# pvangoor/eqf_vio

Measured on AMD Instinct MI355X. Metric: EqF propagate+update steps/sec at N=200 landmarks (fp32); 1-GPU + 8-GPU batch, higher is better.
Workload: dtype f64

## Files before the change

### eqf_vio_amd/csrc/eqf_capi.hip

```cpp
#include <hip/hip_runtime.h>

#include <algorithm>
#include <cmath>
#include <cstdio>
#include <cstdlib>
#include <cstring>
#include <type_traits>
#include <vector>

#include "../../include/eqf_vio_amd_debug.h"
#include "eqf_churn.hpp"
#include "eqf_dense.hpp"
#include "eqf_device.hpp"
#include "eqf_propagate.hpp"
#include "eqf_burst.hpp"
#include "eqf_chol64.hpp"
#include "eqf_resident.hpp"
#include "eqf_update.hpp"
#include "eqf_i8.hpp"
#include "eqf_local.hpp"
#include "eqf_innov.hpp"
#include "eqf_factor.hpp"
#include "eqf_nees.hpp"
#include "eqf_clone.hpp"
#include "eqf_frame.hpp"
#include "eqf_sample.hpp"
#include "eqf_sample_host.hpp"
#include "eqf_blocks.hpp"
#include "eqf_blocks_host.hpp"
#include "eqf_linear.hpp"
#include "eqf_linear_host.hpp"
#include "eqf_mixture.hpp"
#include "eqf_mixture_host.hpp"
#include "eqf_mergecost.hpp"
#include "eqf_mergecost_host.hpp"
#include "eqf_forecast.hpp"
#include "eqf_forecast_host.hpp"
#include "eqf_score.hpp"
#include "eqf_score_host.hpp"
#include "eqf_lift.hpp"
#include "eqf_lift_host.hpp"
#include "eqf_mapedit.hpp"
#include "eqf_mapedit_host.hpp"
#include "eqf_schmidt.hpp"
#include "eqf_schmidt_host.hpp"

using namespace eqf;

#define HIPC(expr)                                                                              \
    do {                                                                                        \
        hipError_t e_ = (expr);                                                                 \
        if (e_ != hipSuccess) {                                                                 \
            std::fprintf(stderr, "eqf_vio_amd: %s failed: %s (%s:%d)\n", #expr, hipGetErrorString(e_), __FILE__, __LINE__); \
            return EQF_ERR_HIP;                                                                 \
        }                                                                                       \
    } while (0)

namespace {
constexpr int kRing = 64;

struct ProfPair {
    int cls, key;
    hipEvent_t a, b;
};
struct ProfSample {
    int key;
    float ms;
};

void launchI8Dd(int slices, const I8DdArgs& a, const UpdArgs* u, int nCt, hipStream_t st) {
    UpdArgs uu{};
    if (u) uu = *u;
    i8WithSlices(slices, [&](auto s) {
        hipLaunchKernelGGL((k_i8dd_split<s>), dim3(nCt + (u ? 1 : 0), a.B), dim3(256), 0, st, a, uu, u ? 1 : 0);
// ... 134 lines not shown
    bool neesLdsSet = false;
    double *dSampZ = nullptr, *dSampE = nullptr;
    int sampRows = 0;
    char *hSampSmall = nullptr, *dSampSmall = nullptr;
    hipEvent_t evSamp = nullptr;
    char *hLinSmall = nullptr, *dLinSmall = nullptr;
    double *dLinWs = nullptr, *dLinOut = nullptr;
    hipEvent_t evLin = nullptr;
    char *hBlkSmall = nullptr, *dBlkSmall = nullptr;
    size_t blkSmallBytes = 0, blkWsDoubles = 0, blkWiInts = 0;
    double *dBlkWs = nullptr, *dBlkOut = nullptr;
    int* dBlkWi = nullptr;
    hipEvent_t evBlk = nullptr;
    bool blkLdsSet = false;
    int liftOpt = 0;
    bool liftCalled = false, liftLdsSet = false;
    double *dLiftRec = nullptr, *dLiftE = nullptr, *dLiftD = nullptr;
    int* dLiftBad = nullptr;
    ClonePair *hClonePairs = nullptr, *dClonePairs = nullptr;
    int clonePairsCap = 0;
    char* dCloneSmall = nullptr;
    hipEvent_t evCloneSrc = nullptr, evCloneDone = nullptr;
    double* dMixWs = nullptr;
    char *hMixTab = nullptr, *dMixTab = nullptr;
    size_t mixTabBytes = 0;
    int mixLaunches = 0;
    hipEvent_t evMix = nullptr;
    int innovStats = 0;
    double* dInnov = nullptr;
    int resTickets = 0;
    double *dGammaPart = nullptr, *dG11Part = nullptr;
    ResRole* dRoles = nullptr;
    int rolesN = -1, rolesCount = 0;
    int rolesFront = 0;
    int dropRole[4] = {-1, 0, 0, 0};
    bool prof = false;
    std::vector<ProfPair> profPairs;
    std::vector<hipEvent_t> evPool;
    long long profCount[EQF_PROF_CLASSES] = {};
    double profMs[EQF_PROF_CLASSES] = {};
    std::vector<ProfSample> profSamples[EQF_PROF_CLASSES];
    double profOverheadMs = 0.0;
    ImuRec *hFcImu = nullptr, *dFcImu = nullptr;
    double *dFcRec = nullptr, *dFcOut = nullptr, *hFcOut = nullptr;
    char* dMcWs = nullptr;
    int mcChunkCap = 0, mcChunkOpt = 0;
    char* dMcItems = nullptr;
    size_t mcItemCap = 0;
    char* dScWs = nullptr;
    int scChunkCap = 0, scChunkOpt = 0;
    char* dScTab = nullptr;
    size_t scTabBytes = 0;
    bool scoreLdsSet = false;
    char *hMapEdit = nullptr, *dMapEdit = nullptr;
    hipEvent_t evMapEdit = nullptr;
    char *hSch = nullptr, *dSch = nullptr;
    char* hSchDev = nullptr;
    hipEvent_t evSch = nullptr;
    bool schLdsSet = false;
};

namespace {

template <typename F>
int profiled(eqf_filter* f, int cls, F&& launch, int key = 0) {
    if (!f->prof) {
// ... 374 lines not shown
        if (status) status[b] = st;
    }
}

UpdArgs makeUpdArgs(eqf_filter* f, const double* bearings, long long bearStride, const int* perm) {
    UpdArgs a{};
    a.g = f->g[f->pG];
    a.p0 = f->p0;
    a.lmc = f->lmc;
    a.Q = f->Q[f->pG];
    a.Sin = f->Sigma[f->pS];
    a.Sout = f->Sigma[f->pS ^ 1];
    a.sigmaStride = f->sigmaStride;
    a.cap = f->cap;
    a.ld = f->ld;
    a.bearings = bearings;
    a.bearStride = bearStride;
    a.perm = perm;
    a.SA = f->SA; a.SL = f->SL; a.YW = f->YW; a.YO = f->YO;
    a.ldS = f->ldS; a.ldY = f->ldY; a.strideS = f->strideS; a.strideY = f->strideY;
    a.EA = f->EA; a.EL = f->EL; a.ZW = f->ZW; a.ZO = f->ZO;
    a.ldE = f->ldE; a.ldZ = f->ldZ; a.strideE = f->strideE; a.strideZ = f->strideZ;
    a.dbgDelta = f->dbgDelta;
    a.dbgGamma = f->dbgGamma;
    a.dbgGammaTot = f->dbgGammaTot;
    a.red = f->red;
    a.errflag = f->errflag;
    a.resCounters = f->dResCounters;
    a.prm = f->prm;
    a.csInBurst = f->csValid ? 1 : 0;
    return a;
}

int buildRoles(eqf_filter* f, int Nmax, bool fold, int front = 0) {
    const int nbS = roundUp(sDim(Nmax), kSB) / kSB, nbE = roundUp(eDim(Nmax), kSB) / kSB, wtS = roundUp(yCols(Nmax), kSB) / kSB;
    const int key = (fold ? 1 << 30 : 0) | (front << 27) | (nbS << 18) | (nbE << 9) | wtS;
    if (f->rolesN == key) return EQF_OK;
    std::vector<ResRole> r;
    if (fold) {
        r.push_back({1, 6, 0, 0});
        r.push_back({0, 6, 0, 0});
        for (int s = 0; s < std::min(front, nbE - 1); ++s) {
            r.push_back({1, 0, s + 1, 0});
            for (int R = s + 2; R < nbE; ++R) r.push_back({1, 1, R, s});
        }
    }
    f->rolesFront = fold ? int(r.size()) : 0;
    if (!(fold && front > 0)) f->rolesFront = 0;
    for (int s = 0; s < std::max(nbS, nbE); ++s)
        for (int kind = 1; kind >= 0; --kind) {
            const int nb = kind ? nbE : nbS, wt = kind ? 1 : wtS;
            if (s >= nb) continue;
            const bool moved = fold && kind == 1 && s < front;
            if (s + 1 < nb && !moved) r.push_back({kind, 0, s + 1, 0});
            for (int R = s + 2; R < nb && !moved; ++R) r.push_back({kind, 1, R, s});
            for (int t = 0; t < wt; ++t) r.push_back({kind, 2, t, s});
        }
    if (f->dropRole[0] >= 0)
        for (auto& q : r)
            if (q.kind == f->dropRole[0] && q.role == f->dropRole[1] && q.R == f->dropRole[2] && q.C == f->dropRole[3]) q.R = 1 << 20;
    HIPC(hipStreamSynchronize(f->stream));
    hipFree(f->dRoles);
    f->dRoles = nullptr;
    int rc = dmalloc(&f->dRoles, r.size());
    if (rc) return rc;
    HIPC(hipMemcpy(f->dRoles, r.data(), sizeof(ResRole) * r.size(), hipMemcpyHostToDevice));
    f->rolesN = key;
    f->rolesCount = int(r.size());
    return EQF_OK;
}

struct UpdateShape {
    int nbS, nbE, wtS, nv;
    int wpb, nvPad, lmBlocks, eBlocks;
    size_t prepLds;
    bool occ2Prep;
    bool embed;
    bool splitChain;
    bool resident;
    bool residentFits;
    bool fold;
    int front;
    bool pipeHeads, occ2;
    int eFromSigma;
    bool small;
    int ddNt, ddTiles;
    int i8Slices;
    bool tailLaunch, tailLift;
};

int updateShape(eqf_filter* f, int Nmax, UpdateShape& s) {
    const int B = f->B;
    const bool f64 = f->precision != EQF_PRECISION_F32;
    s.nbS = roundUp(sDim(Nmax), kSB) / kSB, s.nbE = roundUp(eDim(Nmax), kSB) / kSB, s.wtS = roundUp(yCols(Nmax), kSB) / kSB;
    s.nv = kLm0 + 3 * Nmax;
    const int mp = roundUp(sDim(Nmax), kSB), nep = roundUp(eDim(Nmax), kSB);
    s.nvPad = roundUp(std::min(s.nv, kLm0 + 3 * kPrepLmChunk), 16);
    const size_t perWave = size_t(2) * s.nvPad * sizeof(double);
    s.wpb = int(std::min<size_t>(4, (150 * 1024) / perWave));
    if (s.wpb < 1) return EQF_ERR_CAPACITY;
// ... 47 lines not shown
#endif
    const int fullLds = int(sizeof(Step64Lds));
    auto fn = [](auto* kernel) { return reinterpret_cast<const void*>(kernel); };
    const struct { const void* fn; int bytes; } table[] = {
        {fn(&k_update_prep64<float, false>), prepLds},
        {fn(&k_update_prep64<double, false>), prepLds},
        {fn(&k_update_prep64<float, true>), prepLds},
        {fn(&k_update_prep64<double, true>), prepLds},
        {fn(&k_chol_resident<float, false>), fullLds},
        {fn(&k_chol_resident<double, false>), fullLds},
        {fn(&k_chol_resident<float, true>), fullLds},
        {fn(&k_chol_resident<double, true>), fullLds},
        {fn(&k_chol_resident<float, true, true>), kLdsRes2Bytes},
        {fn(&k_chol_resident<double, true, true>), kLdsRes2Bytes},
        {fn(&k_chol_resident<double, false, false, true>), fullLds},
        {fn(&k_chol_resident<double, true, false, true>), fullLds},
        {fn(&k_chol_resident<double, true, true, true>), kLdsRes2Bytes},
        {fn(&k_chol_resident<float, true, false, false, true>), fullLds},
        {fn(&k_chol_resident<double, true, false, false, true>), fullLds},
        {fn(&k_chol_resident<float, true, true, false, true>), kLdsRes2Bytes},
        {fn(&k_chol_resident<double, true, true, false, true>), kLdsRes2Bytes},
        {fn(&k_chol_step64<float, 0>), fullLds},
        {fn(&k_chol_step64<double, 0>), fullLds},
        {fn(&k_chol_step64<float, 1>), fullLds},
        {fn(&k_chol_step64<double, 1>), fullLds},
        {fn(&k_chol_step64<float, 3>), kLdsTailBytes},
        {fn(&k_chol_step64<double, 3>), kLdsTailBytes},
    };
    for (const auto& e : table) HIPC(hipFuncSetAttribute(e.fn, hipFuncAttributeMaxDynamicSharedMemorySize, e.bytes));
    f->ldsAttrSet = true;
    return EQF_OK;
}

template <typename T>
int launchChainsResident(eqf_filter* f, const UpdateShape& s, const ChainArgs& cS, const ChainArgs& cE, const UpdArgs& a) {
    ResArgs ra{};
    ra.c0 = cS; ra.c1 = cE; ra.a = a;
    ra.roles = f->dRoles;
    ra.readyA = f->dReadyA; ra.readyY = f->dReadyY; ra.counters = f->dResCounters;
    ra.gammaPart = f->dGammaPart; ra.g11Part = f->dG11Part;
    ra.nbCap = f->nbCap; ra.wtCap = f->wtCap;
    ra.stageFlags = f->dStageFlags;
    ra.eFromSigma = s.eFromSigma == 2 ? 1 : 0;
    if (s.fold) {
        ra.waitD0 = 3;
        ra.nPrep = s.lmBlocks + s.eBlocks;
        ra.nFront = f->rolesFront;
        ra.lmBlocks = s.lmBlocks;
        ra.prepWpb = s.wpb;
        ra.prepNvPad = s.nvPad;
        ra.prepFlags = f->dPrepFlags;
        ra.nPrepCap = f->nPrepCap;
    }
    ra.ddNt = s.ddNt;
    ra.nDdTiles = s.i8Slices ? 0 : s.ddTiles;
    ra.nRoles = f->rolesCount;
    ra.errflag = f->errflag;
    const int perFilter = ra.nPrep + f->rolesCount + ra.nDdTiles;
    ra.rolesPerRow = std::min(perFilter, 32768);
    const dim3 rg(f->B * ra.rolesPerRow, (perFilter + ra.rolesPerRow - 1) / ra.rolesPerRow);
    const long long slots = (long long)std::max(f->numCUs, 1) * (s.occ2 ? 2 : 1);
    const bool tickets = f->resTickets == 2 || (f->resTickets == 1 && (long long)rg.x * rg.y >= 6 * slots);
    const bool ticketBuild = s.pipeHeads && !s.fold && tickets && f->dTicket;
    return profiled(f, EQF_PROF_CHOL_RESIDENT, [&] {
        if (ticketBuild) {
            ra.ticket = f->dTicket;
            ra.ticketBase = f->ticketBase;
            f->ticketBase += ra.rolesPerRow * rg.y;
        }
        const dim3 wg(256);
        const size_t fullLds = sizeof(Step64Lds);
        if (s.fold) {
            if constexpr (std::is_same<T, double>::value) {
                if (s.occ2) hipLaunchKernelGGL((k_chol_resident<double, true, true, true>), rg, wg, kLdsRes2Bytes, f->stream, ra);
                else if (s.pipeHeads) hipLaunchKernelGGL((k_chol_resident<double, true, false, true>), rg, wg, fullLds, f->stream, ra);
                else hipLaunchKernelGGL((k_chol_resident<double, false, false, true>), rg, wg, fullLds, f->stream, ra);
// ... 22 lines not shown
        step3Counts(s.nbE, 1, k, &tE, &uE);
        const int nStream = std::min(uS + uE, std::max(1, ((B == 1 ? 4 : 2) * f->numCUs + B - 1) / B));
        rc = profiled(f, dd ? EQF_PROF_CHOL_DD : EQF_PROF_CHOL_STEP, [&] {
            hipLaunchKernelGGL((k_chol_step64<T, 3>), dim3(2 + tS + tE + nStream + dd, B), dim3(256), kLdsTailBytes, f->stream, cS, cE, a, k,
                dd ? s.ddNt : 0, s.small ? 1 : 0, s.embed ? 1 : 0, f->errflag, nStream, 1);
        }, k);
        if (rc) return rc;
    }
    return EQF_OK;
}

template <typename T>
int launchChainsFused(eqf_filter* f, const UpdateShape& s, const ChainArgs& cS, const ChainArgs& cE, const UpdArgs& a) {
    for (int k = 0; k < std::max(s.nbS, s.nbE); ++k) {
        const int dd = (s.embed && k == s.nbS) ? s.ddTiles : 0;
        const int rc = profiled(f, dd ? EQF_PROF_CHOL_DD : EQF_PROF_CHOL_STEP, [&] {
            const int grid = chainBlocks64(s.nbS, s.wtS, k, 0) + chainBlocks64(s.nbE, 1, k, 0);
            hipLaunchKernelGGL((k_chol_step64<T, 0>), dim3(grid + dd, f->B), dim3(256), sizeof(Step64Lds), f->stream, cS, cE, a, k, dd ? s.ddNt : 0,
                s.small ? 1 : 0, s.embed ? 1 : 0, f->errflag);
        }, k);
        if (rc) return rc;
    }
    return EQF_OK;
}

template <typename T>
int launchUpdateT(eqf_filter* f, const double* bearings, long long bearStride, const int* perm, int Nmax) {
    UpdArgs a = makeUpdArgs(f, bearings, bearStride, perm);
    f->csValid = false;
    const int B = f->B;
    UpdateShape s{};
    int rc = allowUpdateLds(f);
    if (!rc) rc = updateShape(f, Nmax, s);
    if (!rc && s.resident) rc = buildRoles(f, Nmax, s.fold, s.front);
    if (rc) return rc;
    a.pad = kSB; a.eFromSigma = s.eFromSigma;
    ChainArgs cS{}, cE{};
    cS.g = a.g; cS.A = f->SA; cS.D = f->SL; cS.W = f->YW; cS.WO = f->YO;
    cS.ldA = f->ldS; cS.ldW = f->ldY; cS.strideA = f->strideS; cS.strideD = f->strideDS; cS.strideW = f->strideY;
    cS.kind = 0; cS.nbMax = s.nbS; cS.wtMax = s.wtS;
    cE.g = a.g; cE.A = f->EA; cE.D = f->EL; cE.W = f->ZW; cE.WO = f->ZO;
    cE.ldA = f->ldE; cE.ldW = f->ldZ; cE.strideA = f->strideE; cE.strideD = f->strideDE; cE.strideW = f->strideZ;
    cE.kind = 1; cE.nbMax = s.nbE; cE.wtMax = 1;
    f->updateEpoch = f->updateEpoch == 0x7fffffff ? 1 : f->updateEpoch + 1;
    cS.flags = f->dFlags; cS.strideF = 2 * f->flagStride; cS.epoch = f->updateEpoch;
    cE.flags = f->dFlags + f->flagStride; cE.strideF = 2 * f->flagStride; cE.epoch = f->updateEpoch;
    if (!s.fold) rc = profiled(f, EQF_PROF_UPDATE_PREP, [&] {
        const dim3 grid(s.lmBlocks + s.eBlocks + 2, B);
        const size_t lds = std::max(s.prepLds, (size_t)kLdsFactorBytes);
        if (s.occ2Prep) hipLaunchKernelGGL((k_update_prep64<T, true>), grid, dim3(256), lds, f->stream, a, cS, cE, s.lmBlocks, s.eBlocks, s.wpb, s.nvPad);
        else hipLaunchKernelGGL((k_update_prep64<T, false>), grid, dim3(256), lds, f->stream, a, cS, cE, s.lmBlocks, s.eBlocks, s.wpb, s.nvPad);
    });
    if (rc) return rc;
    rc = s.resident ? launchChainsResident<T>(f, s, cS, cE, a) : s.splitChain ? launchChainsSplit<T>(f, s, cS, cE, a) : launchChainsFused<T>(f, s, cS, cE, a);
    if (rc) return rc;
    if (s.tailLaunch && s.i8Slices) {
        I8DdArgs ia{};
        ia.Y = a.YO; ia.ldY = a.ldY; ia.strideY = a.strideY;
        ia.Sin = static_cast<const double*>(a.Sin); ia.Sout = static_cast<double*>(a.Sout); ia.ld = a.ld; ia.sigmaStride = a.sigmaStride;
        ia.g = a.g; ia.dims = nullptr; ia.pad = a.pad; ia.skipCol = 11;
        ia.ws = f->dI8Ws; ia.wsStride = f->i8WsStride; ia.expo = f->dI8Expo; ia.expoStride = i8ddExpoWords(kLm0 + 3 * f->cap);
        ia.B = B; ia.nt = (s.nv + 63) / 64;
        rc = profiled(f, EQF_PROF_DOWNDATE, [&] { launchI8Dd(s.i8Slices, ia, s.tailLift ? &a : nullptr, (s.nv + 31) / 32, f->stream); });
    } else if (s.tailLaunch) {
        rc = profiled(f, EQF_PROF_DOWNDATE, [&] {
            if (s.small) hipLaunchKernelGGL((k_downdate<T, 32>), dim3(s.ddTiles + 1, B), dim3(256), (downdateLdsBytes<T, 32>()), f->stream, a, s.ddNt, 1);
            else hipLaunchKernelGGL((k_downdate<T, 64>), dim3(s.ddTiles + 1, B), dim3(256), (downdateLdsBytes<T, 64>()), f->stream, a, s.ddNt, 1);
// ... 180 lines not shown
    ea.gateThr = f->gateThr;
    ea.measVar = f->set.measurementVariance;
    ea.gateFlag = gateArmed ? f->hGateDev : nullptr;
    ea.chordOut = gateArmed ? f->hChordDev : nullptr;
    ea.depthDefault = f->set.initialSceneDepth; ea.pointVar = f->set.initialPointVariance;
    ea.p0 = f->p0; ea.Q = f->Q[f->pG]; ea.lmc = f->lmc;
    ea.errflag = f->errflag;
    ea.Scur = f->Sigma[f->pS]; ea.Soth = f->Sigma[f->pS ^ 1];
    ea.sigmaStride = f->sigmaStride; ea.ld = f->ld;
    ea.hostFlip = anyLost ? 1 : 0;
    ea.bar = f->dEditBar;
    const int coRes = std::max(1, std::min(64, std::max(f->numCUs, 1) / B));
    const int G = (anyLost || !gateArmed) ? std::max(coRes, std::min(1024, (kLm0 + 3 * plan.Nmax + 3) / 4)) : coRes;
    rc = profiled(f, EQF_PROF_CHURN, [&] {
        if (gateArmed && f->gateKind == EQF_GATE_MAHALANOBIS)
            hipLaunchKernelGGL((k_edit<double, 1>), dim3(G, B), dim3(256), 0, f->stream, ea);
        else
            withSigmaType(f, [&](auto t) { hipLaunchKernelGGL((k_edit<decltype(t), 0>), dim3(G, B), dim3(256), 0, f->stream, ea); });
    });
    if (rc) return rc;
    HIPC(hipGetLastError());
    f->ids = std::move(plan.newIds);
    if (status)
        for (int b : plan.skipped) status[b] = EQF_SKIPPED_NO_BEARINGS;
    if (anyLost) f->pS ^= 1;
    f->csValid = false;
    f->permOnDevice.clear();
    if (gateArmed) {
        rc = armGate(f, true, m, bearings, bearStride);
        if (rc) return rc;
        f->gate.nKept = plan.nKept;
    }
    if (!plan.anyWork) return EQF_OK;
    return launchUpdate(f, bearings, bearStride, f->dPerm, plan.Nmax);
}

int gateSpeculatively(eqf_filter* f, const frame::Meas& m, const double* bearings, long long bearStride, const frame::Lists& perm) {
    const int B = f->B;
    frame::Lists permFull = perm;
    for (int b = 0; b < B; ++b)
        if (m.active[b]) frame::forUnmatched(perm[b].data(), int(perm[b].size()), m.n[b], nullptr, [&](int k) { permFull[b].push_back(k); });
    const bool identityPerm = frame::isIdentity(permFull);
    int rc = identityPerm ? EQF_OK : uploadPerm(f, permFull);
    if (!rc) rc = awaitMaskAndClearFlags(f);
    if (!rc) rc = probe(f, bearings, bearStride, !identityPerm, false, true);
    if (!rc) rc = armGate(f, false, m, bearings, bearStride);
    if (rc) return rc;
    f->gate.ids.assign(B, {});
    f->gate.nOld.assign(B, 0);
    for (int b = 0; b < B; ++b) {
        f->gate.ids[b].assign(m.ids[b], m.ids[b] + m.n[b]);
        f->gate.nOld[b] = int(f->ids[b].size());
    }
    f->gate.nb = m.n;
    return EQF_OK;
}

int addNewAndUpdate(eqf_filter* f, const frame::Meas& m, const double* bearings, long long bearStride, int* status, frame::Lists& perm,
    const frame::Marks& dropped, bool depthFresh) {
    const int B = f->B, cap = f->cap;
    bool needDepth = false;
    frame::Lists fresh(B);
    for (int b = 0; b < B; ++b) {
        if (!m.active[b]) continue;
        frame::forUnmatched(perm[b].data(), int(perm[b].size()), m.n[b], dropped[b].data(), [&](int k) { fresh[b].push_back(k); });
        if (!fresh[b].empty()) {
            if (f->ids[b].size() + fresh[b].size() > (size_t)cap) return EQF_ERR_CAPACITY;
// ... 1395 lines not shown
    return EQF_OK;
}

int eqf_debug_option(eqf_filter* f, const char* name, int value) {
    if (!f || !name) return EQF_ERR_INVALID;
    GATE(f);
    if (!std::strcmp(name, "e_sigma_min_percu_x10")) {
        f->eSigmaMinPerCU = value / 10.0;
        return EQF_OK;
    }
    if (!std::strcmp(name, "burst_fused_max_x10")) {
        f->fusedMaxPerCU = value / 10.0;
        return EQF_OK;
    }
    if (!std::strcmp(name, "ring_ahead2")) {
        f->ringAhead2 = value ? 1 : 0;
        return EQF_OK;
    }
    if (!std::strcmp(name, "burst_lm")) {
        if (value != 0 && value != 4 && value != 8 && value != 16) return EQF_ERR_INVALID;
        f->burstLm = value;
        return EQF_OK;
    }
    if (!std::strcmp(name, "burst_rows")) {
        if (value != 0 && value != 1 && value != 2 && value != 4) return EQF_ERR_INVALID;
        f->burstRows = value;
        return EQF_OK;
    }
    if (!std::strcmp(name, "res_tickets")) {
        if (value < 0 || value > 2) return EQF_ERR_INVALID;
        f->resTickets = value;
        return EQF_OK;
    }
    if (!std::strcmp(name, "device_edit")) {
        f->deviceEdit = value ? 1 : 0;
        return EQF_OK;
    }
    if (!std::strcmp(name, "cs_in_burst")) {
        f->csInBurst = value;
        f->csValid = false;
        return EQF_OK;
    }
    return EQF_ERR_INVALID;
}

int eqf_set_option(eqf_filter* f, const char* name, int value) {
    if (!f || !name) return EQF_ERR_INVALID;
    if (!std::strcmp(name, "downdate_slices")) {
        if (value != 0 && (value < 5 || value > 7)) return EQF_ERR_INVALID;
        if (value && f->precision == EQF_PRECISION_F32) return EQF_ERR_UNSUPPORTED;
        GATE(f);
        if (value > f->i8Slices) {
            const int nvCap = kLm0 + 3 * f->cap, mpCap = roundUp(sDim(f->cap), kSB);
            if (!i8Exact(mpCap, value)) return EQF_ERR_CAPACITY;
            HIPC(hipStreamSynchronize(f->stream));
            hipFree(f->dI8Ws);
            hipFree(f->dI8Expo);
            f->dI8Ws = nullptr;
            f->dI8Expo = nullptr;
            f->i8Slices = 0;
            f->ddSlices = 0;
            const long long stride = i8SliceBytes(mpCap, nvCap, value);
            if (hipMalloc(&f->dI8Ws, size_t(stride) * f->B) != hipSuccess ||
                hipMalloc(&f->dI8Expo, sizeof(int) * size_t(i8ddExpoWords(nvCap)) * f->B) != hipSuccess) {
                (void)hipGetLastError();
                hipFree(f->dI8Ws);
// ... 160 lines not shown
    const int B = f->B, nMax = maxN(f);
    if (nrhs > 0 && lde < kBase + 3 * nMax) return EQF_ERR_INVALID;
    int rc = neesAlloc(f);
    if (rc) return rc;
    const int off = first == kBase ? kLm0 : first, ldE = std::max(kLm0 + 3 * nMax - off, 1);
    std::vector<double> hE;
    if (nrhs > 0) {
        hE.assign(size_t(B) * nrhs * ldE, 0.0);
        for (int b = 0; b < B; ++b) {
            const int n = kBase + 3 * int(f->ids[b].size());
            for (int k = 0; k < nrhs; ++k) {
                const double* src = err + (size_t(b) * nrhs + k) * lde;
                double* dst = hE.data() + (size_t(b) * nrhs + k) * ldE;
                for (int i = first; i < n; ++i) dst[(i < kBase ? i : i + 1) - off] = src[i];
            }
        }
        HIPC(hipMemcpyAsync(f->dNeesE, hE.data(), sizeof(double) * hE.size(), hipMemcpyHostToDevice, f->stream));
    }
    rc = neesFactor(f, local, off, nrhs);
    if (rc) return rc;
    std::vector<double> hO(size_t(B) * (kNeesHead + kNeesRhs));
    HIPC(hipMemcpyAsync(hO.data(), f->dNeesOut, sizeof(double) * hO.size(), hipMemcpyDeviceToHost, f->stream));
    HIPC(hipStreamSynchronize(f->stream));
    neesStats(hO.data(), B, stats);
    for (int b = 0; b < B; ++b)
        for (int k = 0; k < nrhs; ++k) nees[size_t(b) * nrhs + k] = hO[size_t(b) * (kNeesHead + kNeesRhs) + kNeesHead + k];
    return EQF_OK;
}

static_assert(lift::kRefBase == kBase && lift::kPadBase == kLm0 && lift::kOff == kLiftOff && lift::kRhs == kLiftRhs && lift::kRec == kLiftRec &&
              lift::kHead == kLiftHead && kLiftHead == kLinHead && lift::kWordFailed == kLiftWordFailed &&
              lift::kWordFailed != blocks::kInfoIdle && lift::kPadPos == kBase - kLiftOff,
    "eqf_lift_host.hpp repeats the layout constants");
namespace {
int liftCallKind(const eqf_filter* f) { return lift::callKind(f->liftOpt, f->prm.useInnovationLift, f->prm.useDiscreteInnovationLift); }
int liftAlloc(eqf_filter* f, bool factors) {
    void *r = nullptr, *e = nullptr, *d = nullptr, *w = nullptr, *s = nullptr;
    bool ok = true;
    if (!f->dLiftRec) ok = hipMalloc(&r, sizeof(double) * size_t(kLiftRec) * f->B) == hipSuccess;
    if (ok && factors && !f->dLiftE)
        ok = hipMalloc(&e, sizeof(double) * lift::rhsDoubles(f->ld) * f->B) == hipSuccess &&
             hipMalloc(&d, sizeof(double) * size_t(kDRec) * f->B) == hipSuccess && hipMalloc(&w, sizeof(int) * size_t(f->B)) == hipSuccess;
    if (ok && factors && !f->dSigmaLoc) ok = hipMalloc(&s, sizeof(double) * size_t(f->sigmaStride) * f->B) == hipSuccess;
    if (!ok) {
        (void)hipGetLastError();
        for (void* p : {r, e, d, w, s})
            if (p) hipFree(p);
        return EQF_ERR_HIP;
    }
    if (r) f->dLiftRec = static_cast<double*>(r);
    if (e) {
        f->dLiftE = static_cast<double*>(e);
        f->dLiftD = static_cast<double*>(d);
        f->dLiftBad = static_cast<int*>(w);
    }
    if (s) f->dSigmaLoc = static_cast<double*>(s);
    return EQF_OK;
}
int liftEnqueue(eqf_filter* f, const double* gamma, long long strideG, int offG, const unsigned char* dMask, double* verdict, bool writesVerdict,
    IncArgs& ia) {
    const int B = f->B, nMax = maxN(f), kind = liftCallKind(f);
    LiftArgs a{};
    a.g = f->g[f->pG]; a.p0 = f->p0; a.Q = f->Q[f->pG]; a.cap = f->cap; a.A = f->dSigmaLoc; a.ld = f->ld; a.strideA = f->sigmaStride;
    a.E = f->dLiftE; a.ldE = lift::rhsPitch(nMax); a.D = f->dLiftD; a.bad = f->dLiftBad; a.gamma = gamma; a.strideG = strideG; a.offG = offG;
    a.mask = dMask; a.verdict = verdict; a.fail = writesVerdict ? verdict : nullptr; a.kind = lift::callFactors(kind, nMax) ? kind : 0;
    a.rec = f->dLiftRec; a.prm = f->prm;
// ... 1214 lines not shown
```

### eqf_vio_amd/csrc/eqf_resident.hpp

```cpp
#pragma once
#include "eqf_chol64.hpp"

namespace eqf {

struct ResRole {
    int kind;
    int role;
    int R, C;
};

struct ResArgs {
    ChainArgs c0, c1;
    UpdArgs a;
    const ResRole* roles;
    int* readyA;
    int* readyY;
    int* counters;
    double* gammaPart;
    double* g11Part;
    int nbCap, wtCap;
    int ddNt;
    int* errflag;
    int nRoles, nDdTiles;
    int rolesPerRow;
    int waitD0;
    int nPrep, lmBlocks, prepWpb, prepNvPad;
    int nFront;
    int* prepFlags;
    int nPrepCap;
    int eFromSigma;
    int* stageFlags;
    unsigned* ticket;
    unsigned ticketBase;
};

EQF_DEV void hoLoadBlocks2(const double* srcA, int ldA, double (*dstA)[kSP], const double* srcB, int ldB, double (*dstB)[kSP], int tid) {
    const int r = tid >> 2, c = (tid & 3) * 16;
    const char* pa = reinterpret_cast<const char*>(srcA + (long long)r * ldA + c);
    const char* pb = reinterpret_cast<const char*>(srcB + (long long)r * ldB + c);
    v4i32 a[8], b[8];
    asm volatile(
        "global_load_dwordx4 %0, %16, off sc0 sc1\n\tglobal_load_dwordx4 %1, %16, off offset:16 sc0 sc1\n\t"
        "global_load_dwordx4 %2, %16, off offset:32 sc0 sc1\n\tglobal_load_dwordx4 %3, %16, off offset:48 sc0 sc1\n\t"
        "global_load_dwordx4 %4, %16, off offset:64 sc0 sc1\n\tglobal_load_dwordx4 %5, %16, off offset:80 sc0 sc1\n\t"
        "global_load_dwordx4 %6, %16, off offset:96 sc0 sc1\n\tglobal_load_dwordx4 %7, %16, off offset:112 sc0 sc1\n\t"
        "global_load_dwordx4 %8, %17, off sc0 sc1\n\tglobal_load_dwordx4 %9, %17, off offset:16 sc0 sc1\n\t"
        "global_load_dwordx4 %10, %17, off offset:32 sc0 sc1\n\tglobal_load_dwordx4 %11, %17, off offset:48 sc0 sc1\n\t"
        "global_load_dwordx4 %12, %17, off offset:64 sc0 sc1\n\tglobal_load_dwordx4 %13, %17, off offset:80 sc0 sc1\n\t"
        "global_load_dwordx4 %14, %17, off offset:96 sc0 sc1\n\tglobal_load_dwordx4 %15, %17, off offset:112 sc0 sc1\n\t"
        "s_waitcnt vmcnt(0)"
        : "=&v"(a[0]), "=&v"(a[1]), "=&v"(a[2]), "=&v"(a[3]), "=&v"(a[4]), "=&v"(a[5]), "=&v"(a[6]), "=&v"(a[7]), "=&v"(b[0]), "=&v"(b[1]),
          "=&v"(b[2]), "=&v"(b[3]), "=&v"(b[4]), "=&v"(b[5]), "=&v"(b[6]), "=&v"(b[7])
        : "v"(pa), "v"(pb)
        : "memory");
#pragma unroll
    for (int u = 0; u < 8; ++u) {
        dstA[r][c + 2 * u] = hoLo(a[u]);
        dstA[r][c + 2 * u + 1] = hoHi(a[u]);
        dstB[r][c + 2 * u] = hoLo(b[u]);
        dstB[r][c + 2 * u + 1] = hoHi(b[u]);
    }
}
EQF_DEV void hoLoadBlock(const double* src, int ld, double (*dst)[kSP], int tid) {
    const int r = tid >> 2, c = (tid & 3) * 16;
    const char* pa = reinterpret_cast<const char*>(src + (long long)r * ld + c);
    v4i32 a[8];
    asm volatile(
// ... 400 lines not shown
    const Glob& g = ch.g[b];
    const bool active = g.updateOk && g.N != 0;
    if (!active) return;
    int nb, wt;
    chainDims64(ch, g.N, &nb, &wt);
    int nbS, wtS, nbE, wtE;
    chainDims64(ra.c0, g.N, &nbS, &wtS);
    chainDims64(ra.c1, g.N, &nbE, &wtE);
    const int tid = threadIdx.x, lane = tid & 63, wv = tid >> 6;
    const int epoch = ch.epoch;
    const Lds64 s = OCC2 ? ldsRes2(smemR) : ldsFull(smemR);
    double* A = ch.A + (long long)b * ch.strideA;
    double* D = ch.D + (long long)b * ch.strideD;
    double* W = ch.W + (long long)b * ch.strideW;
    double* WO = ch.WO + (long long)b * ch.strideW;
    const int ldA = ch.ldA, ldW = ch.ldW;
    const int nbCap = ra.nbCap, wtCap = ra.wtCap;
    int* readyA = ra.readyA + ((long long)b * 2 + role.kind) * nbCap * nbCap;
    int* readyY = ra.readyY + ((long long)b * 2 + role.kind) * nbCap * wtCap;
    const int* flagD = ch.flags + (long long)b * ch.strideF;
    int* counters = ra.counters + (long long)b * 4;
    int bad = 0;
    const bool srcSigma = ra.eFromSigma && role.kind == 1;
    const T* Sg = static_cast<const T*>(a.Sin) + (long long)b * a.sigmaStride;
    const int neE = eDim(g.N), ldS = a.ld;
    auto tile0 = [&](int R, int C, int i, int j) __attribute__((always_inline)) {
        if (!srcSigma) return fold ? hoLoad8(A + (long long)(R * kSB + i) * ldA + C * kSB + j) : A[(long long)(R * kSB + i) * ldA + C * kSB + j];
        const int r = R * kSB + i, c = C * kSB + j;
        const bool in = r < neE && c < neE && r != 5 && c != 5;
        const double v = (double)Sg[in ? (long long)(6 + r) * ldS + 6 + c : 0];
        return in ? v : (r == c ? 1.0 : 0.0);
    };

    auto waitPrep = [&]() {
        if (!fold) return;
        for (int i = tid; i < ra.nPrep; i += 256)
            if (!hoWait(ra.prepFlags + (long long)b * ra.nPrepCap + i, epoch, ra.errflag)) bad = 8;
        bad = __syncthreads_or(bad) ? 8 : 0;
    };
    const bool waitD0 = (ra.waitD0 >> role.kind) & 1;

    if (role.role == 6) {
        factorFirstFromSigma<T, true>(a, ch, b, s, &bad);
        hoDrain();
        __syncthreads();
        if (tid == 0) hoPublish(ch.flags + (long long)b * ch.strideF, epoch);
    } else if (role.role == 0) {
        const int R = role.R;
        if (R >= nb) return;
        int tr[4], tc[4], nt;
        nt = wv >= 2 ? 4 : 1;
        tr[0] = wv; tc[0] = 0;
        tr[1] = wv == 2 ? 1 : 2; tc[1] = 1;
        tr[2] = wv == 2 ? 3 : 2; tc[2] = wv == 2 ? 1 : 2;
        tr[3] = 3;               tc[3] = wv == 2 ? 2 : 3;
        if (!srcSigma) waitPrep();
        f64x4 a1[4], a2[4];
#pragma unroll
        for (int i = 0; i < 4; ++i)
#pragma unroll
            for (int q = 0; q < 4; ++q) {
                a1[i][q] = tile0(R, R - 1, kQB * wv + (lane >> 4) + 4 * q, kQB * i + (lane & 15));
                a2[i][q] = i < nt ? tile0(R, R, kQB * tr[i] + (lane >> 4) + 4 * q, kQB * tc[i] + (lane & 15)) : 0.0;
            }
        EQF_HSTAMP(0);
        if constexpr (PIPEH) {
            if (R > 2) {
                __shared__ int sAheadH;
                PanelRegs pr;
                const double* rowP = A + (long long)(R * kSB) * ldA;
                const double* rowQ = A + (long long)((R - 1) * kSB) * ldA;
                const int nK = R - 2;
                hoWait3(readyA + R * nbCap, readyA + (R - 1) * nbCap, nullptr, epoch, tid, &bad, ra.errflag);
                panelIssue(pr, rowP, ldA, rowQ, ldA, tid);
                bool probe = (tid == 0 && nK > 1) ? hoProbe2(readyA + R * nbCap + 1, readyA + (R - 1) * nbCap + 1, epoch) : false;
                for (int K = 0; K < nK; ++K) {
                    panelToLds(pr, s.P, s.Q, tid);
                    if (tid == 0) sAheadH = probe ? 1 : 0;
                    __syncthreads();
                    const bool ahead = K + 1 < nK && sAheadH;
                    if (ahead) {
                        panelIssue(pr, rowP + (K + 1) * kSB, ldA, rowQ + (K + 1) * kSB, ldA, tid);
                        probe = (tid == 0 && K + 2 < nK) ? hoProbe2(readyA + R * nbCap + K + 2, readyA + (R - 1) * nbCap + K + 2, epoch) : false;
                    }
#pragma unroll
                    for (int i = 0; i < 4; ++i) a1[i] = mmTile<true, kSB>(a1[i], &s.P[0][0], kSP, kQB * wv, &s.Q[0][0], kSP, kQB * i, lane, -1.0);
#pragma unroll
                    for (int i = 0; i < 4; ++i)
                        if (i < nt) a2[i] = mmTile<true, kSB>(a2[i], &s.P[0][0], kSP, kQB * tr[i], &s.P[0][0], kSP, kQB * tc[i], lane, -1.0);
                    __syncthreads();
                    if (K + 1 < nK && !ahead) {
                        hoWait3(readyA + R * nbCap + K + 1, readyA + (R - 1) * nbCap + K + 1, nullptr, epoch, tid, &bad, ra.errflag);
                        panelIssue(pr, rowP + (K + 1) * kSB, ldA, rowQ + (K + 1) * kSB, ldA, tid);
                        probe = (tid == 0 && K + 2 < nK) ? hoProbe2(readyA + R * nbCap + K + 2, readyA + (R - 1) * nbCap + K + 2, epoch) : false;
                    }
                }
            }
// ... 32 lines not shown
        if (R - 1 == 0 || !ra.stageFlags) {
            hoWait3((R - 1 > 0 || waitD0) ? flagD + (R - 1) : nullptr, nullptr, nullptr, epoch, tid, &bad, ra.errflag);
            EQF_HSTAMP(2);
            hoLoadRecord(D + (long long)(R - 1) * kDRec, s, tid);
#pragma unroll
            for (int i = 0; i < 4; ++i) stTile(a1[i], &s.P[0][0], kSP, kQB * wv, kQB * i, lane);
            __syncthreads();
            EQF_HSTAMP(3);
            solveStrip<true>(&s.P[0][0], kSP, s, kQB * wv, lane);
            __syncthreads();
        } else {
            stagedPanelSolve(a1, s, D + (long long)(R - 1) * kDRec, ra.stageFlags + (((long long)b * 2 + role.kind) * nbCap + (R - 1)) * 4,
                flagD + (R - 1), epoch, tid, &bad, ra.errflag);
        }
        EQF_HSTAMP(4);
        hoStoreBlock(A + (long long)(R * kSB) * ldA + (R - 1) * kSB, ldA, s.P, tid);
        a2[0] = mmTile<true, kSB>(a2[0], &s.P[0][0], kSP, kQB * tr[0], &s.P[0][0], kSP, kQB * tc[0], lane, -1.0);
        __syncthreads();
        EQF_HSTAMP(5);
        stTile(a2[0], &s.L[0][0], kSP, kQB * tr[0], kQB * tc[0], lane);
        if (wv == 0) stTile(a2[0], &s.D0[0][0], kWP, 0, 0, lane);
        if (wv == 1) factorPrologueW(s, lane);
        __syncthreads();
        auto pre = [&](int, int r, int c, f64x4& t) {
#pragma unroll
            for (int i = 1; i < 4; ++i)
                if (tr[i] == r && tc[i] == c) t = mmTile<true, kSB>(a2[i], &s.P[0][0], kSP, kQB * tr[i], &s.P[0][0], kSP, kQB * tc[i], lane, -1.0);
        };
        EQF_HSTAMP(6);
        auto mid = [&] {
            if (bad != 8) hoPublish(readyA + R * nbCap + (R - 1), epoch);
            EQF_HSTAMP(12);
        };
        factor64<true>(s, tid, &bad, pre, D + (long long)R * kDRec, EQF_F64_ST(), realStages(ch.kind == 0 ? sDim(g.N) : eDim(g.N), kSB * R), mid,
            stageOut, epoch);
        EQF_HSTAMP(7);
        hoDrain();
        __syncthreads();
        if (tid == 0 && bad != 8) hoPublish(ch.flags + (long long)b * ch.strideF + R, epoch);
        EQF_HSTAMP(8);
    } else if (role.role == 1) {
        const int R = role.R, C = role.C;
        if (R >= nb) return;
        if (!srcSigma) waitPrep();
        f64x4 acc[4];
#pragma unroll
        for (int i = 0; i < 4; ++i)
#pragma unroll
            for (int q = 0; q < 4; ++q) acc[i][q] = tile0(R, C, kQB * wv + (lane >> 4) + 4 * q, kQB * i + (lane & 15));
        if (C > 0) {
            __shared__ int sAhead;
            PanelRegs pr;
            const double* rowP = A + (long long)(R * kSB) * ldA;
            const double* rowQ = A + (long long)(C * kSB) * ldA;
            hoWait3(readyA + R * nbCap, readyA + C * nbCap, nullptr, epoch, tid, &bad, ra.errflag);
            panelIssue(pr, rowP, ldA, rowQ, ldA, tid);
            bool probe = (tid == 0 && C > 1) ? hoProbe2(readyA + R * nbCap + 1, readyA + C * nbCap + 1, epoch) : false;
            for (int K = 0; K < C; ++K) {
                panelToLds(pr, s.P, s.Q, tid);
                if (tid == 0) sAhead = probe ? 1 : 0;
                __syncthreads();
                const bool ahead = K + 1 < C && sAhead;
                if (ahead) {
                    panelIssue(pr, rowP + (K + 1) * kSB, ldA, rowQ + (K + 1) * kSB, ldA, tid);
                    probe = (tid == 0 && K + 2 < C) ? hoProbe2(readyA + R * nbCap + K + 2, readyA + C * nbCap + K + 2, epoch) : false;
                }
#pragma unroll
                for (int i = 0; i < 4; ++i) acc[i] = mmTile<true, kSB>(acc[i], &s.P[0][0], kSP, kQB * wv, &s.Q[0][0], kSP, kQB * i, lane, -1.0);
                __syncthreads();
                if (K + 1 < C && !ahead) {
                    hoWait3(readyA + R * nbCap + K + 1, readyA + C * nbCap + K + 1, nullptr, epoch, tid, &bad, ra.errflag);
                    panelIssue(pr, rowP + (K + 1) * kSB, ldA, rowQ + (K + 1) * kSB, ldA, tid);
                    probe = (tid == 0 && K + 2 < C) ? hoProbe2(readyA + R * nbCap + K + 2, readyA + C * nbCap + K + 2, epoch) : false;
                }
            }
        }
#ifndef EQF_T_STAGED
#define EQF_T_STAGED 1
#endif
        if (EQF_T_STAGED && C > 0 && C + 2 == R && ra.stageFlags) {
            stagedPanelSolve(acc, s, D + (long long)C * kDRec, ra.stageFlags + (((long long)b * 2 + role.kind) * nbCap + C) * 4, flagD + C, epoch, tid, &bad,
                ra.errflag);
        } else {
            hoWait3((C > 0 || waitD0) ? flagD + C : nullptr, nullptr, nullptr, epoch, tid, &bad, ra.errflag);
            hoLoadRecord(D + (long long)C * kDRec, s, tid);
#pragma unroll
            for (int i = 0; i < 4; ++i) stTile(acc[i], &s.P[0][0], kSP, kQB * wv, kQB * i, lane);
            __syncthreads();
            solveStrip<true>(&s.P[0][0], kSP, s, kQB * wv, lane);
            __syncthreads();
        }
        hoStoreBlock(A + (long long)(R * kSB) * ldA + C * kSB, ldA, s.P, tid);
        hoDrain();
        __syncthreads();
        if (tid == 0 && bad != 8) hoPublish(readyA + R * nbCap + C, epoch);
        if (C + 2 == R) EQF_HSTAMP(11);
    } else {
        const int t = role.R, C = role.C;
        if (t >= wt || C >= nb) return;
        const double* Tg = W + (long long)(C * kSB) * ldW + t * kSB;
        waitPrep();
        f64x4 acc[4];
#pragma unroll
        for (int i = 0; i < 4; ++i)
#pragma unroll
            for (int q = 0; q < 4; ++q) {
                const double* p = Tg + (long long)(kQB * wv + (lane >> 4) + 4 * q) * ldW + kQB * i + (lane & 15);
                acc[i][q] = fold ? hoLoad8(p) : *p;
            }
        const bool isS = ch.kind == 0;
        double* zv = s.redL;
        const int nvv = kLm0 + 3 * g.N;
        const bool last = ch.kind == 1 && C == nb - 1;
        const bool lastFast = last && !PIPEH;
        bool collected = false;
        auto collect = [&]() {
            collected = true;
            const int* ryS = ra.readyY + ((long long)b * 2 + 0) * nbCap * wtCap;
            if (tid < wtS && !hoWait(ryS + (nbS - 1) * wtCap + tid, epoch, ra.errflag)) bad = 8;
            bad = __syncthreads_or(bad) ? 8 : 0;
            double* gam = a.dbgGamma + (long long)b * (kLm0 + 3 * a.cap);
            const int ldY = ra.c0.ldW;
            double gv[4];
#pragma unroll
            for (int u = 0; u < 4; ++u) {
                const int col = tid + 256 * u;
                gv[u] = col < nvv + 6 ? hoLoad8(ra.gammaPart + ((long long)b * nbCap + nbS - 1) * ldY + col) : 0.0;
            }
            for (int col = tid + 1024; col < nvv + 6; col += 256) {
                const double v = hoLoad8(ra.gammaPart + ((long long)b * nbCap + nbS - 1) * ldY + col);
                if (col < nvv) gam[col] = v;
                else s.redL[col - nvv] = v;
            }
#pragma unroll
            for (int u = 0; u < 4; ++u) {
                const int col = tid + 256 * u;
                if (col < nvv) gam[col] = col == 11 ? 0.0 : gv[u];
                else if (col < nvv + 6) s.redL[col - nvv] = gv[u];
            }
            if (lastFast) {
                __syncthreads();
                updateFinishBody(a, b, s.redL, 1);
            }
        };
        if (isS && tid < kSB) zv[tid] = fold ? hoLoad8(W + (long long)(C * kSB + tid) * ldW + 11) : W[(long long)(C * kSB + tid) * ldW + 11];
        if (C > 0) {
            __shared__ int sAheadW;
            PanelRegs pr;
            double zNext = 0.0;
            const double* rowQ = A + (long long)(C * kSB) * ldA;
            const double* colP = WO + t * kSB;
            auto issue = [&](int K) {
                panelIssue(pr, colP + (long long)(K * kSB) * ldW, ldW, rowQ + K * kSB, ldA, tid);
                if (isS && tid < kSB) zNext = hoLoad8(WO + (long long)(K * kSB + tid) * ldW + 11);
            };
            auto look = [&](int K) {
                return (tid == 0 && K < C) ? hoProbe3(readyA + C * nbCap + K, readyY + K * wtCap + t, isS ? readyY + K * wtCap : nullptr, epoch) : false;
            };
            auto issueSplit = [&](int K) {
                hoWait3(readyA + C * nbCap + K, nullptr, nullptr, epoch, tid, &bad, ra.errflag);
                panelIssueQ(pr, rowQ + K * kSB, ldA, tid);
                hoWait3(readyY + K * wtCap + t, isS ? readyY + K * wtCap : nullptr, nullptr, epoch, tid, &bad, ra.errflag);
                panelIssueP(pr, colP + (long long)(K * kSB) * ldW, ldW, tid);
                if (isS && tid < kSB) zNext = hoLoad8(WO + (long long)(K * kSB + tid) * ldW + 11);
            };
            issueSplit(0);
            bool probe = look(1);
            for (int K = 0; K < C; ++K) {
                panelToLds(pr, s.P, s.Q, tid);
                if (isS && tid < kSB) zv[kSB + tid] = zNext;
                if (tid == 0) sAheadW = probe ? 1 : 0;
                __syncthreads();
                const bool ahead = K + 1 < C && sAheadW;
                if (ahead) {
                    issue(K + 1);
                    probe = look(K + 2);
                }
// ... 93 lines not shown
```

Measured before the change: 65330.

## Border the last E-chain block to compute Schur complement directly in resident Cholesky

Adds a bordering mode to the resident Cholesky update chains. The 11 RHS rows are embedded as extra rows of the last E block, and the head role writes the 11x11 Schur complement to g11Part. This removes the separate triangular-solve (role 2) work for the E chain on all but the last block, and the host omits those roles via a mask built from per-batch landmark counts. It only applies to non-F32, non-pipeHeads, non-i8 resident paths. It adds branching and a dependency on exact counts, which are disabled when gating is armed.

```diff
diff --git a/eqf_vio_amd/csrc/eqf_border_host.hpp b/eqf_vio_amd/csrc/eqf_border_host.hpp
--- /dev/null
+++ b/eqf_vio_amd/csrc/eqf_border_host.hpp
@@ -0,0 +1,43 @@
+#pragma once
+
+namespace eqf::border {
+
+constexpr int kBlock = 64;
+constexpr int kStage = 16;
+constexpr int kRows = 11;
+constexpr int kMaxStage = 3;
+
+inline int eOrder(int N) { return 6 + 3 * N; }
+inline int sOrder(int N) { return 2 * N; }
+inline int rhsColumns(int N) { return 12 + 3 * N + 6; }
+inline int blocks(int n) { return (n + kBlock - 1) / kBlock; }
+inline int lastStages(int N) {
+    const int rem = eOrder(N) - kBlock * (blocks(eOrder(N)) - 1);
+    const int st = (rem + kStage - 1) / kStage;
+    return st < 1 ? 1 : (st > 4 ? 4 : st);
+}
+inline int borderStage(int N) {
+    const int nst = lastStages(N);
+    return nst <= kMaxStage ? nst : -1;
+}
+inline bool borderOn(int N) { return N > 0 && borderStage(N) >= 0 && blocks(eOrder(N)) >= 2; }
+inline int borderRow(int N, int q) { return kBlock * (blocks(eOrder(N)) - 1) + kStage * borderStage(N) + q; }
+
+inline int chainRoles(int nb, int wt) { return (nb - 1) + (nb - 1) * (nb - 2) / 2 + wt * nb; }
+inline int rolesPlain(int N) { return chainRoles(blocks(sOrder(N)), blocks(rhsColumns(N))) + chainRoles(blocks(eOrder(N)), 1); }
+inline int rolesBorder(int N) { return borderOn(N) ? rolesPlain(N) - (blocks(eOrder(N)) - 1) : rolesPlain(N); }
+
+inline unsigned long long omitMask(const int* counts, int B, int nbMax) {
+    if (nbMax < 2 || nbMax > 62) return 0ull;
+    unsigned long long need = 0ull;
+    for (int b = 0; b < B; ++b) {
+        if (counts[b] <= 0) continue;
+        const int nb = blocks(eOrder(counts[b]));
+        if (nb > nbMax) return 0ull;
+        if (borderOn(counts[b])) need |= 1ull << (nb - 1);
+        else need |= (1ull << nb) - 1ull;
+    }
+    return ~need & ((1ull << nbMax) - 1ull);
+}
+
+}
diff --git a/eqf_vio_amd/csrc/eqf_capi.hip b/eqf_vio_amd/csrc/eqf_capi.hip
--- a/eqf_vio_amd/csrc/eqf_capi.hip
+++ b/eqf_vio_amd/csrc/eqf_capi.hip
@@ -40,6 +40,7 @@
 #include "eqf_score_host.hpp"
 #include "eqf_lift.hpp"
 #include "eqf_lift_host.hpp"
+#include "eqf_border_host.hpp"
 #include "eqf_mapedit.hpp"
 #include "eqf_mapedit_host.hpp"
 #include "eqf_schmidt.hpp"
@@ -240,6 +241,9 @@
     double *dGammaPart = nullptr, *dG11Part = nullptr;
     ResRole* dRoles = nullptr;
     int rolesN = -1, rolesCount = 0;
+    unsigned long long rolesOmit = 0;
+    int resBorder = 1;
+    bool countsExact = true;
     int rolesFront = 0;
     int dropRole[4] = {-1, 0, 0, 0};
     bool prof = false;
@@ -680,10 +684,16 @@
     return a;
 }
 
-int buildRoles(eqf_filter* f, int Nmax, bool fold, int front = 0) {
+int buildRoles(eqf_filter* f, int Nmax, bool fold, int front = 0, bool border = false) {
     const int nbS = roundUp(sDim(Nmax), kSB) / kSB, nbE = roundUp(eDim(Nmax), kSB) / kSB, wtS = roundUp(yCols(Nmax), kSB) / kSB;
     const int key = (fold ? 1 << 30 : 0) | (front << 27) | (nbS << 18) | (nbE << 9) | wtS;
-    if (f->rolesN == key) return EQF_OK;
+    unsigned long long omit = 0;
+    if (border && f->countsExact) {
+        std::vector<int> counts(f->B);
+        for (int b = 0; b < f->B; ++b) counts[b] = int(f->ids[b].size());
+        omit = border::omitMask(counts.data(), f->B, nbE);
+    }
+    if (f->rolesN == key && f->rolesOmit == omit) return EQF_OK;
     std::vector<ResRole> r;
     if (fold) {
         r.push_back({1, 6, 0, 0});
@@ -702,7 +712,8 @@
             const bool moved = fold && kind == 1 && s < front;
             if (s + 1 < nb && !moved) r.push_back({kind, 0, s + 1, 0});
             for (int R = s + 2; R < nb && !moved; ++R) r.push_back({kind, 1, R, s});
-            for (int t = 0; t < wt; ++t) r.push_back({kind, 2, t, s});
+            for (int t = 0; t < wt; ++t)
+                if (!(kind == 1 && ((omit >> s) & 1ull))) r.push_back({kind, 2, t, s});
         }
     if (f->dropRole[0] >= 0)
         for (auto& q : r)
@@ -714,6 +725,7 @@
     if (rc) return rc;
     HIPC(hipMemcpy(f->dRoles, r.data(), sizeof(ResRole) * r.size(), hipMemcpyHostToDevice));
     f->rolesN = key;
+    f->rolesOmit = omit;
     f->rolesCount = int(r.size());
     return EQF_OK;
 }
@@ -827,6 +839,10 @@
     return EQF_OK;
 }
 
+bool useBorder(const eqf_filter* f, const UpdateShape& s) {
+    return f->resBorder && s.resident && !s.pipeHeads && f->precision != EQF_PRECISION_F32 && !s.i8Slices;
+}
+
 template <typename T>
 int launchChainsResident(eqf_filter* f, const UpdateShape& s, const ChainArgs& cS, const ChainArgs& cE, const UpdArgs& a) {
     ResArgs ra{};
@@ -837,6 +853,7 @@
     ra.nbCap = f->nbCap; ra.wtCap = f->wtCap;
     ra.stageFlags = f->dStageFlags;
     ra.eFromSigma = s.eFromSigma == 2 ? 1 : 0;
+    ra.border = useBorder(f, s) ? 1 : 0;
     if (s.fold) {
         ra.waitD0 = 3;
         ra.nPrep = s.lmBlocks + s.eBlocks;
@@ -925,7 +942,7 @@
     UpdateShape s{};
     int rc = allowUpdateLds(f);
     if (!rc) rc = updateShape(f, Nmax, s);
-    if (!rc && s.resident) rc = buildRoles(f, Nmax, s.fold, s.front);
+    if (!rc && s.resident) rc = buildRoles(f, Nmax, s.fold, s.front, useBorder(f, s));
     if (rc) return rc;
     a.pad = kSB; a.eFromSigma = s.eFromSigma;
     ChainArgs cS{}, cE{};
@@ -1172,7 +1189,10 @@
         f->gate.nKept = plan.nKept;
     }
     if (!plan.anyWork) return EQF_OK;
-    return launchUpdate(f, bearings, bearStride, f->dPerm, plan.Nmax);
+    f->countsExact = !gateArmed;
+    rc = launchUpdate(f, bearings, bearStride, f->dPerm, plan.Nmax);
+    f->countsExact = true;
+    return rc;
 }
 
 int gateSpeculatively(eqf_filter* f, const frame::Meas& m, const double* bearings, long long bearStride, const frame::Lists& perm) {
@@ -2634,6 +2654,11 @@
         f->resTickets = value;
         return EQF_OK;
     }
+    if (!std::strcmp(name, "res_border")) {
+        if (value != 0 && value != 1) return EQF_ERR_INVALID;
+        f->resBorder = value;
+        return EQF_OK;
+    }
     if (!std::strcmp(name, "device_edit")) {
         f->deviceEdit = value ? 1 : 0;
         return EQF_OK;
@@ -2860,6 +2885,7 @@
               lift::kHead == kLiftHead && kLiftHead == kLinHead && lift::kWordFailed == kLiftWordFailed &&
               lift::kWordFailed != blocks::kInfoIdle && lift::kPadPos == kBase - kLiftOff,
     "eqf_lift_host.hpp repeats the layout constants");
+static_assert(border::kBlock == kSB && border::kStage == kQB && border::kRows == kBorderRows, "eqf_border_host.hpp repeats the layout constants");
 namespace {
 int liftCallKind(const eqf_filter* f) { return lift::callKind(f->liftOpt, f->prm.useInnovationLift, f->prm.useDiscreteInnovationLift); }
 int liftAlloc(eqf_filter* f, bool factors) {
diff --git a/eqf_vio_amd/csrc/eqf_resident.hpp b/eqf_vio_amd/csrc/eqf_resident.hpp
--- a/eqf_vio_amd/csrc/eqf_resident.hpp
+++ b/eqf_vio_amd/csrc/eqf_resident.hpp
@@ -32,7 +32,14 @@
     int* stageFlags;
     unsigned* ticket;
     unsigned ticketBase;
+    int border;
 };
+
+constexpr int kBorderRows = 11;
+EQF_DEV int borderStageOf(int ne, int nb) {
+    const int nst = realStages(ne, kSB * (nb - 1));
+    return nst <= 3 ? nst : -1;
+}
 
 EQF_DEV void hoLoadBlocks2(const double* srcA, int ldA, double (*dstA)[kSP], const double* srcB, int ldB, double (*dstB)[kSP], int tid) {
     const int r = tid >> 2, c = (tid & 3) * 16;
@@ -499,6 +506,24 @@
         return in ? v : (r == c ? 1.0 : 0.0);
     };
 
+    const int bst = (!PIPEH && ra.border && nbE >= 2) ? borderStageOf(neE, nbE) : -1;
+    const bool borderRole = bst >= 0 && role.kind == 1;
+    auto borderTile = [&](f64x4& v, int C, int tr16, int c0) __attribute__((always_inline)) {
+        if (tr16 != bst) return;
+        const double* Zw = ra.c1.W + (long long)b * ra.c1.strideW;
+        const int c = C * kSB + c0 + (lane & 15);
+        const bool in = c < neE && c != 5;
+#pragma unroll
+        for (int q = 0; q < 4; ++q) {
+            const int rr = (lane >> 4) + 4 * q;
+            if (rr < kBorderRows) {
+                const double* p = Zw + (in ? (long long)c * ra.c1.ldW + rr : 0);
+                const double z = fold ? hoLoad8(p) : *p;
+                v[q] = in ? z : 0.0;
+            }
+        }
+    };
+
     auto waitPrep = [&]() {
         if (!fold) return;
         for (int i = tid; i < ra.nPrep; i += 256)
@@ -521,7 +546,8 @@
         tr[1] = wv == 2 ? 1 : 2; tc[1] = 1;
         tr[2] = wv == 2 ? 3 : 2; tc[2] = wv == 2 ? 1 : 2;
         tr[3] = 3;               tc[3] = wv == 2 ? 2 : 3;
-        if (!srcSigma) waitPrep();
+        const bool borderHead = borderRole && R == nb - 1;
+        if (!srcSigma || borderHead) waitPrep();
         f64x4 a1[4], a2[4];
 #pragma unroll
         for (int i = 0; i < 4; ++i)
@@ -530,6 +556,13 @@
                 a1[i][q] = tile0(R, R - 1, kQB * wv + (lane >> 4) + 4 * q, kQB * i + (lane & 15));
                 a2[i][q] = i < nt ? tile0(R, R, kQB * tr[i] + (lane >> 4) + 4 * q, kQB * tc[i] + (lane & 15)) : 0.0;
             }
+        if (borderHead) {
+#pragma unroll
+            for (int i = 0; i < 4; ++i) {
+                borderTile(a1[i], R - 1, wv, kQB * i);
+                if (i < nt) borderTile(a2[i], R, tr[i], kQB * tc[i]);
+            }
+        }
         EQF_HSTAMP(0);
         if constexpr (PIPEH) {
             if (R > 2) {
@@ -628,22 +661,45 @@
             if (bad != 8) hoPublish(readyA + R * nbCap + (R - 1), epoch);
             EQF_HSTAMP(12);
         };
-        factor64<true>(s, tid, &bad, pre, D + (long long)R * kDRec, EQF_F64_ST(), realStages(ch.kind == 0 ? sDim(g.N) : eDim(g.N), kSB * R), mid,
-            stageOut, epoch);
+        factor64<true>(s, tid, &bad, pre, borderHead ? nullptr : D + (long long)R * kDRec, EQF_F64_ST(),
+            realStages(ch.kind == 0 ? sDim(g.N) : eDim(g.N), kSB * R), mid, stageOut, epoch);
         EQF_HSTAMP(7);
-        hoDrain();
-        __syncthreads();
-        if (tid == 0 && bad != 8) hoPublish(ch.flags + (long long)b * ch.strideF + R, epoch);
-        EQF_HSTAMP(8);
+        if (borderHead) {
+            if (wv == (bst == 1 ? 2 : 3)) {
+                f64x4 t = bst == 1 ? a2[1] : (bst == 2 ? a2[2] : a2[3]);
+                t = mmTile<true, kSB>(t, &s.P[0][0], kSP, kQB * bst, &s.P[0][0], kSP, kQB * bst, lane, -1.0);
+                for (int j = 0; j < bst; ++j) t = mmTile<true, kQB>(t, &s.L[0][kQB * j], kSP, kQB * bst, &s.L[0][kQB * j], kSP, kQB * bst, lane, -1.0);
+                double* gOut = ra.g11Part + ((long long)b * nbCap + R) * 128;
+#pragma unroll
+                for (int q = 0; q < 4; ++q) {
+                    const int rr = (lane >> 4) + 4 * q, cc = lane & 15;
+                    if (rr < kBorderRows && cc < kBorderRows) hoStore8(gOut + rr * kBorderRows + cc, -t[q]);
+                }
+            }
+            hoDrain();
+            __syncthreads();
+            if (tid == 0 && bad != 8) hoPublish(readyY + R * wtCap, epoch);
+            EQF_HSTAMP(8);
+        } else {
+            hoDrain();
+            __syncthreads();
+            if (tid == 0 && bad != 8) hoPublish(ch.flags + (long long)b * ch.strideF + R, epoch);
+            EQF_HSTAMP(8);
+        }
     } else if (role.role == 1) {
         const int R = role.R, C = role.C;
         if (R >= nb) return;
-        if (!srcSigma) waitPrep();
+        const bool borderT = borderRole && R == nb - 1;
+        if (!srcSigma || borderT) waitPrep();
         f64x4 acc[4];
 #pragma unroll
         for (int i = 0; i < 4; ++i)
 #pragma unroll
             for (int q = 0; q < 4; ++q) acc[i][q] = tile0(R, C, kQB * wv + (lane >> 4) + 4 * q, kQB * i + (lane & 15));
+        if (borderT) {
+#pragma unroll
+            for (int i = 0; i < 4; ++i) borderTile(acc[i], C, wv, kQB * i);
+        }
         if (C > 0) {
             __shared__ int sAhead;
             PanelRegs pr;
@@ -694,6 +750,7 @@
     } else {
         const int t = role.R, C = role.C;
         if (t >= wt || C >= nb) return;
+        if (borderRole && C != nb - 1) return;
         const double* Tg = W + (long long)(C * kSB) * ldW + t * kSB;
         waitPrep();
         f64x4 acc[4];
@@ -702,7 +759,7 @@
 #pragma unroll
             for (int q = 0; q < 4; ++q) {
                 const double* p = Tg + (long long)(kQB * wv + (lane >> 4) + 4 * q) * ldW + kQB * i + (lane & 15);
-                acc[i][q] = fold ? hoLoad8(p) : *p;
+                acc[i][q] = borderRole ? 0.0 : (fold ? hoLoad8(p) : *p);
             }
         const bool isS = ch.kind == 0;
         double* zv = s.redL;
@@ -739,6 +796,22 @@
                 updateFinishBody(a, b, s.redL, 1);
             }
         };
+        if (borderRole) {
+            collect();
+            EQF_WSTAMP(0);
+            hoWait3(readyY + C * wtCap, nullptr, nullptr, epoch, tid, &bad, ra.errflag);
+            EQF_WSTAMP(1);
+            if (tid < 121) s.redL[8 + tid] = hoLoad8(ra.g11Part + ((long long)b * nbCap + C) * 128 + tid);
+            if (__syncthreads_or(tid == 0 && bad == 8)) {
+                if (ra.errflag && tid == 0) atomicOr(ra.errflag, kHoErrTimeout);
+                return;
+            }
+            EQF_WSTAMP(4);
+            updateFinishBody(a, b, s.redL, lastFast ? 2 : 0);
+            __syncthreads();
+            EQF_WSTAMP(5);
+            return;
+        }
         if (isS && tid < kSB) zv[tid] = fold ? hoLoad8(W + (long long)(C * kSB + tid) * ldW + 11) : W[(long long)(C * kSB + tid) * ldW + 11];
         if (C > 0) {
             __shared__ int sAheadW;
```

Measured after the change: 67310, median of 6. 1.03x the previous value.
